# gabormarko/3D-semantic-segmentation

Measured on AMD Instinct MI355X. Metric: Mvoxel-views/sec, higher is better.
Workload: dtype f32; 1 GPU; R2: 200000 voxels x 300 views x 968x548x512 fp32 feature maps, room-shell scene seed 0, dmin 0.01 dmax 10 step 0.5*voxel; views_per_call=60, resident_feature_maps=60, parallelism=single GPU

## Files before the change

### 3d-semantic-segmentation_amd/csrc/voxproj.hip

```cpp
#include <hip/hip_runtime.h>

#include <cmath>
#include <cstdarg>
#include <cstdint>
#include <cstdio>
#include <cstdlib>
#include <cstring>
#include <algorithm>
#include <chrono>
#include <mutex>
#include <unordered_map>
#include <vector>

#include "voxproj.h"

#include "vp_common.h"
#include "vp_tables.h"
#include "vp_march.h"
#include "vp_gather.h"
#include "vp_aux.h"
#include "vp_prep.h"
#include "vp_aggregate.h"
#include "vp_render.h"
#include "vp_query.h"
#include "vp_splat.h"

#define VP_DISPATCH_KVU(KERNEL, VEC_OK, C, ...)                                   \
    do {                                                                          \
        if ((VEC_OK) == 2) hipLaunchKernelGGL((KERNEL<1, 8, VP_F16_U>), __VA_ARGS__);    \
        else if ((VEC_OK) && (C) > 256) hipLaunchKernelGGL((KERNEL<2, 4, 4>), __VA_ARGS__); \
        else if (VEC_OK) hipLaunchKernelGGL((KERNEL<1, 4, 4>), __VA_ARGS__);      \
        else hipLaunchKernelGGL((KERNEL<4, 1, 4>), __VA_ARGS__);                  \
    } while (0)
#define VP_DISPATCH_GATHER(G32, VEC_OK, C, ...)                                   \
    do {                                                                          \
        if ((VEC_OK) == 2) hipLaunchKernelGGL((k_gather<1, 8, VP_F16_U, GATHER_G16>), __VA_ARGS__);    \
        else if ((VEC_OK) && (C) > 256) hipLaunchKernelGGL((k_gather<2, 4, 4, G32>), __VA_ARGS__); \
        else if (VEC_OK) hipLaunchKernelGGL((k_gather<1, 4, 4, G32>), __VA_ARGS__);      \
        else hipLaunchKernelGGL((k_gather<4, 1, 4, 1>), __VA_ARGS__);               \
    } while (0)

#define VP_DISPATCH_GATHER_ONE(SMALL, VEC_OK, C, ...)                             \
    do {                                                                          \
        if ((VEC_OK) == 2) hipLaunchKernelGGL((k_gather_one<1, 8, VP_F16_U>), __VA_ARGS__);    \
        else if ((VEC_OK) && (C) > 256 && (SMALL)) hipLaunchKernelGGL((k_gather_one<2, 4, 8>), __VA_ARGS__); \
        else if ((VEC_OK) && (C) > 256) hipLaunchKernelGGL((k_gather_one<2, 4, 4>), __VA_ARGS__); \
        else if (VEC_OK) hipLaunchKernelGGL((k_gather_one<1, 4, 4>), __VA_ARGS__);      \
        else hipLaunchKernelGGL((k_gather_one<4, 1, 4>), __VA_ARGS__);                  \
    } while (0)

#ifndef VP_F16_U
#define VP_F16_U 4
#endif

extern "C" {

int vp_abi_version(void) { return VP_ABI_VERSION; }

const char *vp_last_error(void) { return g_err; }

size_t vp_workspace_bytes(int B, int V, int H, int W, int C, int dimz, int dimy, int dimx, int64_t n_rows)
{
    if (B <= 0 || V <= 0 || H <= 0 || W <= 0 || C <= 0 || n_rows <= 0 || dimz <= 0 || dimy <= 0 || dimx <= 0) return 0;
    return make_layout(B, V, H, W, C, n_rows, dimz, dimy, dimx).total;
}

static int workspace_status_impl(void *workspace, void *stream_, bool drain_all);

static int project_impl(const float *feats, bool feats_f16, const int64_t *occ, const float *vmi, const float *intr,
                        const float *opts_host, int32_t *count, float *out, int32_t *views_hit,
                        const float *grid_origin_host, float voxel_size,
                        int B, int V, int H, int W, int C, int dimz, int dimy, int dimx, int64_t n_rows,
                        void *workspace, size_t workspace_bytes, void *stream_, int flags, int32_t *ids_out = nullptr)
{
    const bool march_only = ids_out != nullptr;
    if (feats_f16 && (C % 8 != 0 || ((uintptr_t)feats & 15) != 0 || ((uintptr_t)out & 15) != 0))
        return fail(VP_EINVAL, "fp16 feature maps need C %% 8 == 0 and 16-byte aligned feats/out");
    if ((!march_only && (!feats || !count || !out)) || !occ || !vmi || !intr || !opts_host || !grid_origin_host || !workspace)
        return fail(VP_EINVAL, "null pointer argument");
    WsState *st = ws_state(workspace, true);
    struct HitGuard { WsState *st; bool keep; ~HitGuard() { if (!keep) st->has_hit = false; } } hit_guard{st, false};
    if (B <= 0 || V <= 0 || H <= 0 || W <= 0 || C <= 0 || dimz <= 0 || dimy <= 0 || dimx <= 0 || n_rows <= 0)
        return fail(VP_EINVAL, "non-positive dimension");
    if ((long long)B * V > 65535) return fail(VP_EINVAL, "B*V = %lld exceeds 65535", (long long)B * V);
    if ((long long)dimz * dimy * dimx >= (1ll << 31)) return fail(VP_EINVAL, "occupancy grid has >= 2^31 cells per batch");
    if ((long long)H * W >= (1ll << 31) || n_rows >= (1ll << 31)) return fail(VP_EINVAL, "image or row count >= 2^31");
    if ((flags & VP_FLAG_SYNC) && (flags & VP_FLAG_PIPELINE)) return fail(VP_EINVAL, "VP_FLAG_SYNC and VP_FLAG_PIPELINE exclude each other");
    Params p;
    p.width = (int)(opts_host[0] + 0.5f);
    p.height = (int)(opts_host[1] + 0.5f);
    if (p.width != W || p.height != H)
        return fail(VP_EINVAL, "opts width/height (%d,%d) must equal the feature map's (%d,%d)", p.width, p.height, W, H);
    p.dmin = opts_host[2]; p.dmax = opts_host[3]; p.inc = opts_host[4];
    if (!(p.inc > 0.0f)) return fail(VP_EINVAL, "rayIncrement must be > 0 (the reference would never terminate)");
    p.ox = grid_origin_host[0]; p.oy = grid_origin_host[1]; p.oz = grid_origin_host[2];
    p.vs = voxel_size;
    p.dimz = dimz; p.dimy = dimy; p.dimx = dimx;
    p.B = B; p.V = V; p.C = C; p.n_rows = n_rows;

    const Layout l = make_layout(B, V, H, W, C, n_rows, dimz, dimy, dimx, workspace_bytes);
    if (workspace_bytes < l.total) return fail(VP_EWORKSPACE, "workspace has %zu bytes, need %zu", workspace_bytes, l.total);
    if ((uintptr_t)workspace & 255) return fail(VP_EWORKSPACE, "workspace must be 256-byte aligned");
    if (!sticky_open(*st)) return fail(VP_EHIP, "could not allocate the workspace record's page of pinned host memory (sticky error words)");
    char *ws = (char *)workspace;
    hipStream_t s0 = (hipStream_t)stream_;

    const bool pipe = (flags & VP_FLAG_PIPELINE) != 0;
    PipeState *ps = &st->pipe;
    if (pipe && !pipe_open(*ps)) return fail(VP_EHIP, "could not create the side stream / events for VP_FLAG_PIPELINE");
    const bool gather_only = (flags & VP_FLAG_GATHER_ONLY) != 0;
    if (gather_only) {
        if (!st->has_hit || st->last_feats != (const void *)feats || st->last_f16 != feats_f16 || st->last_B != B || st->last_V != V ||
            st->last_H != H || st->last_W != W || st->last_C != C || st->B != B || st->dimz != dimz || st->dimy != dimy ||
            st->dimx != dimx || st->n_rows != n_rows || st->last_out != (const void *)out || st->last_count != (const void *)count ||
            st->last_vmi != (const void *)vmi)
            return fail(VP_EINVAL, "VP_FLAG_GATHER_ONLY repeats phase 2 of the previous call on this workspace: there is none (or it "
                                   "failed), or its feature maps / poses / outputs / shapes differ from this call's");
        if (st->opt_row_begin < 0 && st->opt_row_end < 0)
            return fail(VP_EINVAL, "VP_FLAG_GATHER_ONLY without a row range (VP_OPT_ROW_BEGIN / VP_OPT_ROW_END) would gather every row twice");
        if (!st->last_ranged)
            return fail(VP_EINVAL, "VP_FLAG_GATHER_ONLY after a call that had no row range: that call gathered every row already");
    }

    int q = 0;
    hipStream_t s1 = s0;
    if (gather_only) {
        q = st->last_q;
    } else if (pipe) {
        q = (int)(ps->calls & 1);
        s1 = ps->side;
    } else if (ps->ok && (ps->used[0] || ps->used[1])) {
        VP_HIP(hipStreamSynchronize(ps->side));
        ps->used[0] = ps->used[1] = false;
    }
    int *status = (int *)(ws + l.status[q]);
    int *cell_of_id = (int *)(ws + l.cell_of_id);
    unsigned long long *mask64 = (unsigned long long *)(ws + l.mask64);
    NearRec *near2 = (NearRec *)(ws + l.near2);
    unsigned char *dist = (unsigned char *)(ws + l.dist);
    unsigned char *dist_tmp = (unsigned char *)(ws + l.dist_tmp);
    int *cnt_call = (int *)(ws + l.cnt_call[q]);
    int *heavy_list = (int *)(ws + l.heavy[q]);
    int *work = (int *)(ws + l.work[q]);
    ViewEntry *viewtab = (ViewEntry *)(ws + l.viewtab[q]);
    int *hit = (int *)(ws + l.hit[q]);
    int *status0 = (int *)(ws + l.status[0]);

    const long long cells = (long long)dimz * dimy * dimx;
    int *occ_copy = (int *)(ws + l.occ_copy);
    WsState &rec = *st;
    const bool rec_matches = rec.B == B && rec.dimz == dimz && rec.dimy == dimy && rec.dimx == dimx && rec.n_rows == n_rows;
    const bool verify = (flags & VP_FLAG_VERIFY_ACCEL) && !pipe && !gather_only && !(flags & VP_FLAG_REUSE_ACCEL);
    const int cmp_blocks = (int)((cells * B + 255) / 256 > 8192 ? 8192 : (cells * B + 255) / 256);
    bool rebuild = !gather_only && !(flags & VP_FLAG_REUSE_ACCEL);
    if (!rebuild && !gather_only && (rec.builds == 0 || !rec_matches))
        return fail(VP_EINVAL, "VP_FLAG_REUSE_ACCEL, but this workspace holds no occupancy tables for a grid of this shape "
                               "(B, dims, n_rows): call once without the flag");
    if (rebuild || !rec.opened) {
        if (pipe && ps->ok) {
            VP_HIP(hipStreamSynchronize(ps->side));
        }
        hipLaunchKernelGGL(k_ws_open, dim3(1), dim3(64), 0, s0, status0, (int *)(ws + l.status[1]), WS_MAGIC, rec.gen, rebuild ? 1 : 0);
        rec.opened = true;
    }
    if (verify && rec_matches && rec.copy_valid) {
        volatile int *differs = rec.sticky_host + ST_OCCDIFF;
        *differs = 0;
        hipLaunchKernelGGL(k_occ_compare_copy, dim3(cmp_blocks), dim3(256), 0, s0, (const long long *)occ, occ_copy, cells * B, rec.sticky_dev + ST_OCCDIFF);
        VP_HIP(hipStreamSynchronize(s0));
        rebuild = *differs != 0;
    } else if (rebuild) {
        if (verify) {
            hipLaunchKernelGGL(k_occ_compare_copy, dim3(cmp_blocks), dim3(256), 0, s0, (const long long *)occ, occ_copy, cells * B, status + ST_OCCDIFF);
            rec.copy_valid = true;
        } else {
            rec.copy_valid = false;
        }
    }
    if (rebuild) {
        if (pipe) {
            VP_HIP(hipStreamSynchronize(ps->side));
            VP_HIP(hipStreamSynchronize(s0));
        }
        ProfSpan sp; sp.begin(0, s0);
        VP_HIP(hipMemsetAsync(cell_of_id, 0xFF, size_t(B) * n_rows * sizeof(int), s0));
        VP_HIP(hipMemsetAsync(mask64, 0, size_t(B) * l.nblk * sizeof(unsigned long long), s0));
        const int blocks = (int)((cells * B + 255) / 256 > 16384 ? 16384 : (cells * B + 255) / 256);
        hipLaunchKernelGGL(k_build_cells, dim3(blocks), dim3(256), 0, s0, (const long long *)occ, cell_of_id,
                           mask64, dimz, dimy, dimx, l.nby, l.nbx, l.nblk, B, (long long)n_rows);
        const int db = (int)(((long long)l.nbz * l.nby * l.nbx * B + 255) / 256);
        hipLaunchKernelGGL(k_block_dist, dim3(db), dim3(256), 0, s0, mask64, (const unsigned char *)nullptr, dist, l.nbz, l.nby, l.nbx, l.nblk, B, 0);
        hipLaunchKernelGGL(k_block_dist, dim3(db), dim3(256), 0, s0, mask64, (const unsigned char *)dist, dist_tmp, l.nbz, l.nby, l.nbx, l.nblk, B, 1);
        hipLaunchKernelGGL(k_block_dist, dim3(db), dim3(256), 0, s0, mask64, (const unsigned char *)dist_tmp, dist, l.nbz, l.nby, l.nbx, l.nblk, B, 2);
        const long long near_waves = (long long)l.nbz * l.nby * l.nbx * B;
        hipLaunchKernelGGL(k_build_near, dim3((unsigned)((near_waves + 3) / 4)), dim3(256), 0, s0, mask64, (const unsigned char *)dist,
                           near2, dimz, dimy, dimx, l.nbz, l.nby, l.nbx, l.nblk, B);
        rec.B = B; rec.dimz = dimz; rec.dimy = dimy; rec.dimx = dimx; rec.n_rows = n_rows;
        rec.builds++;
        hipLaunchKernelGGL(k_ws_seal, dim3(1), dim3(1), 0, s0, status0, tables_key(B, dimz, dimy, dimx, n_rows, rec.builds));
        sp.end();
        if (pipe) VP_HIP(hipStreamSynchronize(s0));
    }
    const unsigned expect_tables = tables_key(rec.B, rec.dimz, rec.dimy, rec.dimx, rec.n_rows, rec.builds);

    if (pipe && !gather_only) {
        if (ps->used[q]) VP_HIP(hipStreamWaitEvent(s1, ps->call_done[q], 0));
    }
    const bool ranged = rec.opt_row_begin >= 0 || rec.opt_row_end >= 0;
    const long long row_lo = std::max<long long>(1, rec.opt_row_begin);
    const long long row_hi = rec.opt_row_end < 0 ? (long long)n_rows : std::min<long long>(rec.opt_row_end, (long long)n_rows);

    int heavy_t = (int)std::min<long long>(256 + 64ll * B * V, 2048);
    if ((long long)B * V == 1) heavy_t = 256 + 64;
    if (rec.opt_heavy_t > 0) heavy_t = (int)std::min<long long>(rec.opt_heavy_t, 2147483647ll);
    if (flags & VP_FLAG_SERIAL_SUMS) heavy_t = 2147483647;
    const bool one_view = (long long)B * V == 1 && rec.opt_one_view != 0;
    PlanArgs plan;
    plan.heavy_t = heavy_t; plan.part_t = 2147483647; plan.part_px = 0; plan.count_heavy = 1; plan.dyn_px_min = 0; plan.dyn_t_ratio = 0;
    plan.dyn_t_floor = 0; plan.cell_in_item = 0;
    const long long px2 = 2ll * B * V * (long long)H * W;
    const bool one_split = one_view && heavy_t != 2147483647 && rec.opt_one_view_split != 0;
    if (!one_view && heavy_t != 2147483647) {
        long long ppx = rec.opt_part_px > 0 ? rec.opt_part_px : std::max<long long>(1, heavy_t);
        ppx = std::max(ppx, (px2 + l.slot_cap - 1) / l.slot_cap);
        plan.part_px = (int)std::min<long long>(ppx, 2147483647ll);
        heavy_t = std::max(heavy_t, plan.part_px);
        plan.heavy_t = plan.part_t = heavy_t;
    } else if (one_split) {
        const long long T = rec.opt_one_view_split > 0 ? rec.opt_one_view_split : rec.opt_heavy_t > 0 ? rec.opt_heavy_t : 0;
        long long ppx = rec.opt_part_px > 0 ? std::max(rec.opt_part_px, (px2 + l.slot_cap - 1) / l.slot_cap) : 0;
        if (ppx == 0 && T > 0) ppx = std::max<long long>((T + ONE_VIEW_T_RATIO - 1) / ONE_VIEW_T_RATIO, (px2 + l.slot_cap - 1) / l.slot_cap);
        plan.part_px = (int)std::min<long long>(ppx, 2147483646ll);
        plan.dyn_px_min = ppx > 0 ? 0 : ONE_VIEW_PART_MIN;
        plan.heavy_t = plan.part_t = T > 0 ? (int)std::min<long long>(std::max(T, ppx), 2147483646ll) : 0;
        plan.dyn_t_ratio = T > 0 ? 0 : ONE_VIEW_T_RATIO;
        plan.dyn_t_floor = (long long)H * W <= GATHER_G32_SMALL_IMAGE ? ONE_VIEW_T_FLOOR_SMALL : 0;
        plan.cell_in_item = 1;
        heavy_t = plan.heavy_t;
    } else if (one_view) {
        plan.count_heavy = 0;
    }
    static_assert(sizeof(PlanArgs) == sizeof(int) * 8, "PlanArgs is kept as ints in the workspace record");
    if (gather_only) { memcpy(&plan, st->last_plan, sizeof(plan)); heavy_t = plan.heavy_t; }
    const int part_px = plan.part_px;
    const bool plans_parts = part_px > 0 || plan.dyn_px_min > 0;
#ifdef VP_DIAG
    if (flags & VP_FLAG_DIAG_EVALS) heavy_t = -1;
    if (flags & VP_FLAG_DIAG_WAVES) heavy_t = -2;
#endif
    const int wl_blocks = (int)((n_rows + 256 * WL_PER_THREAD - 1) / (256 * WL_PER_THREAD));
    int4 *parts = (int4 *)(ws + l.parts[q]), *split = (int4 *)(ws + l.split[q]), *pmeta = (int4 *)(ws + l.pmeta[q]);
    float *prow = (float *)(ws + l.prow[q]);
    int *hit_waves = (int *)(ws + l.hitcnt[q]);
#define VP_LAUNCH_WORKLIST(STREAM)                                                                                              \
    hipLaunchKernelGGL(k_worklist, dim3((unsigned)(wl_blocks + (B * V + 255) / 256)), dim3(256), 0, STREAM, (const int *)cnt_call,   \
                       plan, (long long)n_rows, work, status, wl_blocks, vmi, viewtab, B * V, row_lo, row_hi, parts, split, \
                       (int)l.slot_cap, rec.sticky_dev, (const int *)cell_of_id, (const int *)hit_waves, (int)l.n_hitcnt)
    if (gather_only) {
        VP_HIP(hipMemsetAsync(status + ST_WORK0, 0, ST_PLAN_WORDS * sizeof(int), s0));
        VP_LAUNCH_WORKLIST(s0);
    }
    if (!gather_only) {
        ProfSpan sp; sp.begin(0, s1);
        hipLaunchKernelGGL(k_zero_call, dim3((unsigned)((n_rows + 1023) / 1024)), dim3(256), 0, s1, status, cnt_call, (long long)n_rows,
                           status0, rec.sticky_dev, WS_MAGIC, rec.gen, expect_tables, hit_waves,
                           (plan.dyn_px_min > 0 && !march_only) ? l.n_hitcnt : 0ll);
        sp.end();
    }
    if (!gather_only) {
        FirstHitArgs fa;
        fa.occ = (const long long *)occ; fa.vmi = vmi; fa.intr = intr; fa.near2 = near2; fa.dist = dist;
        fa.nby = l.nby; fa.nbx = l.nbx; fa.nblk = l.nblk; fa.hit = march_only ? (int *)ids_out : hit; fa.cnt_call = cnt_call;
        fa.heavy_list = heavy_list; fa.heavy_t = ((one_view && !one_split) || heavy_t < 0) ? heavy_t : 2147483647;
        fa.hit_waves = (plan.dyn_px_min > 0 && l.n_hitcnt > 0) ? hit_waves : nullptr;
        if (march_only) { fa.heavy_t = 2147483647; fa.hit_waves = nullptr; }
        fa.status = status; fa.sticky = rec.sticky_dev;
        const dim3 grid((W + 15) / 16, (H + 15) / 16, B * V);
        ProfSpan sp; sp.begin(1, s1);
        if (flags & VP_FLAG_EXACT_MARCH) {
            hipLaunchKernelGGL(k_first_hit<0>, grid, dim3(256), 0, s1, fa, p);
        } else {
            bool beside_gather = false;
            if (pipe && ps->used[q ^ 1]) {
                beside_gather = hipEventQuery(ps->call_done[q ^ 1]) == hipErrorNotReady;
                (void)hipGetLastError();
            }
            const size_t row_bytes = size_t(C) * (feats_f16 ? 2 : 4);
            size_t lds_req = beside_gather ? (row_bytes <= 1024 ? 30 : 41) * 1024 : 0;
            if (rec.opt_march_lds_kb >= 0) lds_req = size_t(std::min<long long>(rec.opt_march_lds_kb, 64)) * 1024;
            hipLaunchKernelGGL(k_first_hit<1>, grid, dim3(256), lds_req, s1, fa, p);
        }
        if (!march_only) VP_LAUNCH_WORKLIST(s1);
        sp.end();
    }
    if (march_only) {
        VP_HIP(hipGetLastError());
        ps->last_q = 0;
        if (flags & VP_FLAG_SYNC) return workspace_status_impl(workspace, stream_, true);
        return VP_OK;
    }
    if (pipe && !gather_only) VP_HIP(hipEventRecord(ps->fh_done[q], s1));

    GatherArgs g;
    g.feats = feats; g.hit = hit; g.viewtab = viewtab; g.intr = intr; g.cell_of_id = cell_of_id;
    g.cnt_call = cnt_call; g.heavy_list = heavy_list; g.n_heavy = status + ST_NHEAVY;
    g.row_lo = (int)row_lo; g.row_hi = (int)row_hi;
    g.work = work; g.work_n = status + ST_WORK0;
    g.parts = parts; g.split = split; g.pmeta = pmeta; g.prow = prow;
    g.host_word = nullptr; g.host_seq = 0;
    g.parts_on = (one_view && plans_parts) ? 1 : 0; g.slot_cap = (int)l.slot_cap; g.count = count; g.views_hit = views_hit; g.out = out; g.status = status;
    const int vec_ok = feats_f16 ? 2 : ((C % 4 == 0) && (((uintptr_t)feats & 15) == 0) && (((uintptr_t)out & 15) == 0)) ? 1 : 0;
    const bool small_image = (long long)B * V >= 8 && (long long)H * W <= GATHER_G32_SMALL_IMAGE;
    g.heavy_blocks = 0;
    if (pipe && !gather_only) VP_HIP(hipStreamWaitEvent(s0, ps->fh_done[q], 0));
    if (one_view) {
        ProfSpan sp; sp.begin(2, s0);
        const int per_cu = rec.opt_one_view > 0 ? (int)std::min<long long>(rec.opt_one_view, 256) : 16;
        const long long want = rec.opt_one_view >= 1000 ? rec.opt_one_view - 1000 : (long long)device_cus() * per_cu;
        const long long cap = (n_rows - 1 + 3) / 4;
        const unsigned nblk = (unsigned)std::max<long long>(1, std::min(want, cap));
        g.heavy_blocks = (heavy_t != 2147483647 && !plans_parts) ? (int)nblk : 0;
        volatile int *note = nullptr;
        if ((flags & VP_FLAG_SYNC) && plans_parts && n_rows > 1) {
            rec.split_seq = (rec.split_seq + 1) & 0x7fffu;
            note = rec.sticky_host + ST_HOST_NSPLIT;
            *note = 0;
            g.host_word = rec.sticky_dev + ST_HOST_NSPLIT; g.host_seq = (int)rec.split_seq;
        }
        if (n_rows > 1) VP_DISPATCH_GATHER_ONE((long long)H * W <= GATHER_G32_SMALL_IMAGE, vec_ok, C, dim3(nblk), dim3(256), 0, s0, g, p);
        sp.end();
        bool combine = n_rows > 1 && plans_parts;
        if (combine && note) {
            const auto t0 = std::chrono::steady_clock::now();
            for (unsigned spin = 0;; spin++) {
                const unsigned v = (unsigned)*note;
                if ((v >> 31) && ((v >> 16) & 0x7fffu) == rec.split_seq) { combine = (v & 0xffffu) != 0; break; }
                if ((spin & 63) == 63 && std::chrono::steady_clock::now() - t0 > std::chrono::milliseconds(2)) break;
                __builtin_ia32_pause();
            }
        }
        if (combine) {
            ProfSpan sc; sc.begin(3, s0);
            const dim3 cgrid((unsigned)std::max<long long>(1, std::min<long long>(COMBINE_BLOCKS, l.slot_cap / 2)));
            VP_DISPATCH_KVU(k_combine_parts, vec_ok, C, cgrid, dim3(256), 0, s0, g, p);
            sc.end();
        }
    } else if (n_rows > 1) {
        const long long items = (n_rows - 1) + (part_px > 0 ? std::min<long long>(l.slot_cap, px2 / part_px + 1) : 0);
        {
            ProfSpan sp; sp.begin(2, s0);
            const dim3 ggrid((unsigned)((items + 3) / 4));
            if (small_image) VP_DISPATCH_GATHER(4, vec_ok, C, ggrid, dim3(256), 0, s0, g, p);
            else VP_DISPATCH_GATHER(1, vec_ok, C, ggrid, dim3(256), 0, s0, g, p);
            sp.end();
        }
        if (part_px > 0) {
            ProfSpan sp; sp.begin(3, s0);
            const dim3 cgrid((unsigned)std::min<long long>(COMBINE_BLOCKS, std::max<long long>(1, l.slot_cap / 2)));
            VP_DISPATCH_KVU(k_combine_parts, vec_ok, C, cgrid, dim3(256), 0, s0, g, p);
            sp.end();
        }
    }
    if (pipe) {
        VP_HIP(hipEventRecord(ps->call_done[q], s0));
        ps->used[q] = true;
        ps->last_q = q;
        if (!gather_only) ps->calls++;
    } else if (!gather_only) {
        ps->last_q = 0;
    }
    VP_HIP(hipGetLastError());
    st->last_B = B; st->last_V = V; st->last_H = H; st->last_W = W; st->last_C = C; st->last_q = q;
    st->last_f16 = feats_f16; st->last_feats = (const void *)feats; st->last_out = (const void *)out; st->last_count = (const void *)count;
    st->last_vmi = (const void *)vmi; st->last_ranged = ranged; memcpy(st->last_plan, &plan, sizeof(plan));
    st->has_hit = true; st->hit_off = l.hit[q];
    hit_guard.keep = true;
    if (flags & VP_FLAG_SYNC) return workspace_status_impl(workspace, stream_, true);
    return VP_OK;
}

int vp_project_features(const float *feats, const int64_t *occ, const float *vmi, const float *intr,
                        const float *opts_host, int32_t *count, float *out, int32_t *views_hit,
                        const float *grid_origin_host, float voxel_size,
                        int B, int V, int H, int W, int C, int dimz, int dimy, int dimx, int64_t n_rows,
                        void *workspace, size_t workspace_bytes, void *stream_, int flags)
{
    return project_impl(feats, false, occ, vmi, intr, opts_host, count, out, views_hit, grid_origin_host, voxel_size,
                        B, V, H, W, C, dimz, dimy, dimx, n_rows, workspace, workspace_bytes, stream_, flags);
}

int vp_project_features_f16(const void *feats_f16, const int64_t *occ, const float *vmi, const float *intr,
                            const float *opts_host, int32_t *count, float *out, int32_t *views_hit,
                            const float *grid_origin_host, float voxel_size,
                            int B, int V, int H, int W, int C, int dimz, int dimy, int dimx, int64_t n_rows,
                            void *workspace, size_t workspace_bytes, void *stream_, int flags)
{
    return project_impl((const float *)feats_f16, true, occ, vmi, intr, opts_host, count, out, views_hit,
                        grid_origin_host, voxel_size, B, V, H, W, C, dimz, dimy, dimx, n_rows, workspace,
                        workspace_bytes, stream_, flags);
}

int vp_first_hit_ids(const int64_t *occ, const float *vmi, const float *intr, const float *opts_host,
                     const float *grid_origin_host, float voxel_size, int B, int V, int H, int W,
                     int dimz, int dimy, int dimx, int64_t n_rows, int32_t *ids,
                     void *workspace, size_t workspace_bytes, void *stream_, int flags)
{
    const int allowed = VP_FLAG_SYNC | VP_FLAG_REUSE_ACCEL | VP_FLAG_VERIFY_ACCEL | VP_FLAG_EXACT_MARCH;
    if (flags & ~allowed) return fail(VP_EINVAL, "vp_first_hit_ids accepts VP_FLAG_SYNC, _REUSE_ACCEL, _VERIFY_ACCEL and _EXACT_MARCH only (flags 0x%x)", flags);
    if (!ids) return fail(VP_EINVAL, "null pointer argument");
    return project_impl(nullptr, false, occ, vmi, intr, opts_host, nullptr, nullptr, nullptr, grid_origin_host, voxel_size,
                        B, V, H, W, 1, dimz, dimy, dimx, n_rows, workspace, workspace_bytes, stream_, flags, ids);
}

#ifndef RENDER_MAX_BLOCKS
#define RENDER_MAX_BLOCKS (1 << 20)
#endif

int vp_render_features(const int32_t *ids, int64_t n_pixels, const float *rows, int64_t n_rows, int C, void *dst,
                       int dst_is_f16, int32_t *bad_ids, void *stream_)
{
    if (!ids || !rows || !dst) return fail(VP_EINVAL, "null pointer argument");
    if (n_pixels <= 0 || n_rows <= 0 || C <= 0) return fail(VP_EINVAL, "non-positive dimension (n_pixels, n_rows or C)");
    hipStream_t stream = (hipStream_t)stream_;
    const long long tiles = (n_pixels + 63) / 64;
    const dim3 grid((unsigned)std::min<long long>((tiles + 3) / 4, RENDER_MAX_BLOCKS));
    const bool al16 = (((uintptr_t)rows | (uintptr_t)dst) & 15) == 0;
    int *bad = (int *)bad_ids;
#define VP_RENDER(KERNEL) hipLaunchKernelGGL(KERNEL, grid, dim3(256), 0, stream, (const int *)ids, (long long)n_pixels, rows, \
                                             (long long)n_rows, C, dst_t, bad)
    if (dst_is_f16) {
        _Float16 *dst_t = (_Float16 *)dst;
        if (C < 64) VP_RENDER((k_render_small<_Float16>));
        else if (C % 8 == 0 && al16) VP_RENDER((k_render_walk<8, 1, _Float16>));
        else VP_RENDER((k_render_walk<1, 4, _Float16>));
    } else {
        float *dst_t = (float *)dst;
        if (C < 64) VP_RENDER((k_render_small<float>));
        else if (C % 4 == 0 && al16) VP_RENDER((k_render_walk<4, 2, float>));
        else VP_RENDER((k_render_walk<1, 4, float>));
    }
#undef VP_RENDER
    VP_HIP(hipGetLastError());
    return VP_OK;
}

size_t vp_query_workspace_bytes(int P, int C)
{
    if (P < 1 || P > QUERY_MAX_P || C < 1 || C > QUERY_MAX_C) return 0;
    return align256((size_t)query_ppad(P) * query_cpad(C) * sizeof(float));
}

int vp_query_features(const void *rows, int rows_is_f16, int64_t n_rows, int C, int64_t row_stride, const float *text, int P,
                      float scale, float *logits, int32_t *labels, float *margin, int32_t *n_nonfinite, void *workspace,
                      size_t workspace_bytes, void *stream_)
{
    if (!rows || !labels || !text) return fail(VP_EINVAL, "null pointer argument (rows, labels or text)");
    if (n_rows < 1 || n_rows > INT32_MAX) return fail(VP_EINVAL, "n_rows = %lld outside [1, 2^31 - 1]", (long long)n_rows);
    if (C < 1 || C > QUERY_MAX_C) return fail(VP_EINVAL, "C = %d outside [1, %d]", C, QUERY_MAX_C);
    if (P < 1 || P > QUERY_MAX_P) return fail(VP_EINVAL, "P = %d outside [1, %d]", P, QUERY_MAX_P);
    if (row_stride < C) return fail(VP_EINVAL, "row_stride %lld < C = %d", (long long)row_stride, C);
    if (!(scale > 0.0f) || !std::isfinite(scale)) return fail(VP_EINVAL, "scale must be finite and > 0 (got %g)", (double)scale);
    const size_t need = vp_query_workspace_bytes(P, C);
    if (!workspace || workspace_bytes < need) return fail(VP_EWORKSPACE, "workspace has %zu bytes, need %zu", workspace ? workspace_bytes : 0, need);
    if ((uintptr_t)workspace & 255) return fail(VP_EWORKSPACE, "workspace must be 256-byte aligned");
    hipStream_t stream = (hipStream_t)stream_;
    const size_t esz = rows_is_f16 ? 2 : 4;
    const bool vec = C % (16 / esz) == 0 && ((uintptr_t)rows & 15) == 0 && ((size_t)row_stride * esz) % 16 == 0;
    const dim3 grid((unsigned)((n_rows + 16 * QUERY_WAVES - 1) / (16 * QUERY_WAVES))), block(64 * QUERY_WAVES);
#define VP_QUERY(T, VEC) hipLaunchKernelGGL((k_query<T, VEC, false>), grid, block, 0, stream, (const T *)rows, (long long)n_rows, C, \
                                            (long long)row_stride, (const T *)workspace, P, scale, logits, (int *)labels, margin, \
                                            (int *)n_nonfinite)
#define VP_QUERY1(T) hipLaunchKernelGGL((k_query<T, true, true>), grid, block, 0, stream, (const T *)rows, (long long)n_rows, C, \
                                        (long long)row_stride, (const T *)workspace, P, scale, logits, (int *)labels, margin, \
                                        (int *)n_nonfinite)
    if (rows_is_f16) {
        hipLaunchKernelGGL((k_query_text<_Float16>), dim3(query_ppad(P)), dim3(64), 0, stream, text, P, C, (_Float16 *)workspace);
        if (vec && C <= QUERY_NS * QueryTraits<_Float16>::W) VP_QUERY1(_Float16);
        else if (vec) VP_QUERY(_Float16, true);
        else VP_QUERY(_Float16, false);
    } else {
        hipLaunchKernelGGL((k_query_text<float>), dim3(query_ppad(P)), dim3(64), 0, stream, text, P, C, (float *)workspace);
        if (vec && C <= QUERY_NS * QueryTraits<float>::W) VP_QUERY1(float);
        else if (vec) VP_QUERY(float, true);
        else VP_QUERY(float, false);
    }
#undef VP_QUERY
#undef VP_QUERY1
    VP_HIP(hipGetLastError());
    return VP_OK;
}

size_t vp_splat_workspace_bytes(int64_t n_gaussians, int W, int H, int64_t capacity)
{
    if (n_gaussians < 0 || n_gaussians > INT32_MAX || W < 1 || W > SPLAT_MAX_WH || H < 1 || H > SPLAT_MAX_WH || capacity < 0 ||
        capacity > INT32_MAX)
        return 0;
    SplatLayout l;
    return splat_layout(n_gaussians, W, H, capacity, l) ? l.bytes : 0;
}

int vp_splat_project(const float *means, const float *quats, const float *scales, const float *opacities, int64_t n_gaussians,
                     const float *viewmat, float fx, float fy, float cx, float cy, int W, int H, float near_plane,
                     float far_plane, float eps2d, int64_t *n_isect, int32_t *n_nonfinite, void *workspace,
                     size_t workspace_bytes, void *stream_)
{
    if (n_gaussians < 0 || n_gaussians > INT32_MAX)
        return fail(VP_EINVAL, "n_gaussians = %lld outside [0, 2^31 - 1]", (long long)n_gaussians);
    if (n_gaussians > 0 && (!means || !quats || !scales || !opacities))
        return fail(VP_EINVAL, "null pointer argument (means, quats, scales or opacities)");
    if (!viewmat) return fail(VP_EINVAL, "null viewmat");
    if (W < 1 || W > SPLAT_MAX_WH || H < 1 || H > SPLAT_MAX_WH)
        return fail(VP_EINVAL, "image %d x %d outside [1, %d]^2", W, H, SPLAT_MAX_WH);
    for (int k = 0; k < 12; ++k)
        if (!std::isfinite(viewmat[k])) return fail(VP_EINVAL, "viewmat[%d] is not finite", k);
    if (!(fx > 0.0f) || !(fy > 0.0f) || !std::isfinite(fx) || !std::isfinite(fy) || !std::isfinite(cx) || !std::isfinite(cy))
        return fail(VP_EINVAL, "fx, fy must be finite and > 0, cx, cy finite (got %g %g %g %g)", (double)fx, (double)fy,
                    (double)cx, (double)cy);
    if (!(near_plane > 0.0f) || !(far_plane > near_plane) || !(eps2d >= 0.0f) || !std::isfinite(eps2d))
        return fail(VP_EINVAL, "need 0 < near < far and a finite eps2d >= 0 (got %g %g %g)", (double)near_plane,
                    (double)far_plane, (double)eps2d);
    if (!workspace) return fail(VP_EWORKSPACE, "workspace is NULL");
    if ((uintptr_t)workspace & 255) return fail(VP_EWORKSPACE, "workspace must be 256-byte aligned");
    SplatLayout l;
    if (!splat_layout(n_gaussians, W, H, 0, l)) return fail(VP_EHIP, "rocprim scratch size query failed");
    if (workspace_bytes < l.bytes) return fail(VP_EWORKSPACE, "workspace has %zu bytes, need %zu", workspace_bytes, l.bytes);
    hipStream_t stream = (hipStream_t)stream_;
    char *ws = (char *)workspace;
    SplatCam cam;
    for (int k = 0; k < 12; ++k) cam.r[k] = viewmat[k];
    cam.fx = fx; cam.fy = fy; cam.cx = cx; cam.cy = cy;
    cam.near_z = near_plane; cam.far_z = far_plane; cam.eps2d = eps2d;
    cam.W = W; cam.H = H; cam.tiles_x = l.tiles_x;
    long long *total = (long long *)(ws + l.total), *offs = (long long *)(ws + l.offs);
    if (n_gaussians > 0) {
        hipLaunchKernelGGL(k_splat_project, dim3((unsigned)((n_gaussians + 255) / 256)), dim3(256), 0, stream, means, quats,
                           scales, opacities, (long long)n_gaussians, cam, (SplatRec *)(ws + l.rec), (int4 *)(ws + l.box),
                           (int *)(ws + l.count), (int *)n_nonfinite);
        VP_HIP(hipGetLastError());
        size_t tmp = l.scan_bytes;
        VP_HIP(rocprim::inclusive_scan(ws + l.scan_tmp, tmp, (const int *)(ws + l.count), offs, (size_t)n_gaussians,
                                       rocprim::plus<long long>(), stream));
    }
    hipLaunchKernelGGL(k_splat_total, dim3(1), dim3(1), 0, stream, (const long long *)offs, (long long)n_gaussians, total,
                       (long long *)n_isect);
    VP_HIP(hipGetLastError());
    return VP_OK;
}

int vp_splat_rasterize(const float *features, int D, int64_t row_stride, int64_t n_gaussians, int W, int H, int64_t capacity,
                       int32_t *labels, float *confidence, float *alpha, float *logits, int32_t *status, void *workspace,
                       size_t workspace_bytes, void *stream_)
{
    if (n_gaussians < 0 || n_gaussians > INT32_MAX)
        return fail(VP_EINVAL, "n_gaussians = %lld outside [0, 2^31 - 1]", (long long)n_gaussians);
    if (!labels || (n_gaussians > 0 && !features)) return fail(VP_EINVAL, "null pointer argument (labels or features)");
    if (D < 1 || D > SPLAT_MAX_D) return fail(VP_EINVAL, "D = %d outside [1, %d]", D, SPLAT_MAX_D);
    if (row_stride < D) return fail(VP_EINVAL, "row_stride %lld < D = %d", (long long)row_stride, D);
    if (W < 1 || W > SPLAT_MAX_WH || H < 1 || H > SPLAT_MAX_WH)
        return fail(VP_EINVAL, "image %d x %d outside [1, %d]^2", W, H, SPLAT_MAX_WH);
    if (capacity < 0 || capacity > INT32_MAX) return fail(VP_EINVAL, "capacity = %lld outside [0, 2^31 - 1]", (long long)capacity);
    if (!workspace) return fail(VP_EWORKSPACE, "workspace is NULL");
    if ((uintptr_t)workspace & 255) return fail(VP_EWORKSPACE, "workspace must be 256-byte aligned");
    SplatLayout l;
    if (!splat_layout(n_gaussians, W, H, capacity, l)) return fail(VP_EHIP, "rocprim scratch size query failed");
    if (workspace_bytes < l.bytes) return fail(VP_EWORKSPACE, "workspace has %zu bytes, need %zu", workspace_bytes, l.bytes);
    hipStream_t stream = (hipStream_t)stream_;
    char *ws = (char *)workspace;
    const long long n_tiles = (long long)l.tiles_x * l.tiles_y;
    const long long *total = (const long long *)(ws + l.total);
    unsigned long long *k0 = (unsigned long long *)(ws + l.keys0), *k1 = (unsigned long long *)(ws + l.keys1);
    int *v0 = (int *)(ws + l.vals0), *v1 = (int *)(ws + l.vals1);
    longlong2 *ranges = (longlong2 *)(ws + l.ranges);
    const long long n_emit = std::max<long long>(n_gaussians, 1);
    const unsigned g_emit = (unsigned)((n_emit + 255) / 256);
    hipLaunchKernelGGL(k_splat_emit, dim3(g_emit), dim3(256), 0, stream, (const SplatRec *)(ws + l.rec),
                       (const int4 *)(ws + l.box), (const long long *)(ws + l.offs), (long long)n_gaussians, l.tiles_x,
                       n_tiles, total, (long long)capacity, k0, v0, (int *)status);
    VP_HIP(hipGetLastError());
    if (capacity > 0) {
        size_t tmp = l.sort_bytes;
        VP_HIP(rocprim::radix_sort_pairs(ws + l.sort_tmp, tmp, k0, k1, v0, v1, (size_t)capacity, 0u, (unsigned)l.end_bit,
                                         stream));
    }
    VP_HIP(hipMemsetAsync(ranges, 0, (size_t)n_tiles * sizeof(longlong2), stream));
    if (capacity > 0) {
        hipLaunchKernelGGL(k_splat_ranges, dim3((unsigned)((capacity + 255) / 256)), dim3(256), 0, stream, k1, total,
                           (long long)capacity, ranges);
        VP_HIP(hipGetLastError());
    }
    const dim3 grid((unsigned)l.tiles_x, (unsigned)l.tiles_y), block(SPLAT_THREADS);
#define VP_SPLAT(DT) hipLaunchKernelGGL((k_splat_blend<DT>), grid, block, 0, stream, (const SplatRec *)(ws + l.rec), v1, ranges, \
                                        total, (long long)capacity, features, D, (long long)row_stride, W, H, (int *)labels, \
                                        confidence, alpha, logits)
    if (D <= 8) VP_SPLAT(8);
    else if (D <= 16) VP_SPLAT(16);
    else if (D <= 32) VP_SPLAT(32);
    else VP_SPLAT(64);
#undef VP_SPLAT
    VP_HIP(hipGetLastError());
    return VP_OK;
}

static int read_status(void *workspace, hipStream_t stream, int *st )
{
// ... 324 lines not shown
```

### 3d-semantic-segmentation_amd/csrc/vp_march.h

```cpp
#pragma once

namespace {

struct FirstHitArgs {
    const long long *occ;
    const float *vmi;
    const float *intr;
    const NearRec *near2;
    const unsigned char *dist;
    int nby, nbx;
    long long nblk;
    int *hit;
    int *cnt_call;
    int *heavy_list;
    int heavy_t;
    int *hit_waves;
    int *status;
    int *sticky;
};

struct MarchView {
    const long long *occ_b;
    const NearRec *near_b;
    const unsigned char *dist_b;
    int nby, nbx;
    float cpx, cpy, cpz;
    float fx, fy, mx, my, fw, fh;
    float rvs;
};

struct MarchRay {
    float cdx, cdy, cdz;
    float wdx, wdy, wdz;
    float tEnd;
    float inv_dcell;
    float thr;
    bool leap_ok;
};

struct MarchBlock {
    unsigned cur_blk = 0xffffffffu;
    int cur_d = 0;
    unsigned long long p0 = 0ull, p1 = 0ull, p2 = 0ull;
};

struct MarchBinade {
    float bT2 = 0.0f, bTu = 0.0f, bg = 0.0f, brg = 0.0f;
};

__device__ __forceinline__ int march_sample(const Params &p, const MarchView &mv, const MarchRay &r, MarchBlock &mb, float t, int &D)
{
    const float px = mv.cpx + t * r.wdx, py = mv.cpy + t * r.wdy, pz = mv.cpz + t * r.wdz;
    const float ax = px - p.ox, ay = py - p.oy, az = pz - p.oz;
    const float qx = ax * mv.rvs, qy = ay * mv.rvs, qz = az * mv.rvs;
    const float rx = rintf(qx), ry = rintf(qy), rz = rintf(qz);
    const bool safe = (fabsf(qx - rx) < r.thr) & (fabsf(qy - ry) < r.thr) & (fabsf(qz - rz) < r.thr);
    int ix = (int)rx, iy = (int)ry, iz = (int)rz;
    if (__builtin_expect(!safe, 0)) {
        ix = f2i_sat(round_half_away(ax / p.vs));
        iy = f2i_sat(round_half_away(ay / p.vs));
        iz = f2i_sat(round_half_away(az / p.vs));
    }
    D = 0;
    const bool ing = ((unsigned)ix < (unsigned)p.dimx) & ((unsigned)iy < (unsigned)p.dimy) & ((unsigned)iz < (unsigned)p.dimz);
    if (__builtin_expect(ing, 1)) {
        const unsigned blk = ((unsigned)(iz >> 2) * (unsigned)mv.nby + (unsigned)(iy >> 2)) * (unsigned)mv.nbx + (unsigned)(ix >> 2);
        if (blk != mb.cur_blk) {
            mb.cur_blk = blk;
            const NearRec n3 = mv.near_b[blk];
            mb.cur_d = (int)n3.dist;
            mb.p0 = n3.p0; mb.p1 = n3.p1; mb.p2 = n3.p2;
        }
        const int bit = ((iz & 3) << 4) | ((iy & 3) << 2) | (ix & 3);
        const int nd = (int)((mb.p0 >> bit) & 1ull) | ((int)((mb.p1 >> bit) & 1ull) << 1) | ((int)((mb.p2 >> bit) & 1ull) << 2);
        D = mb.cur_d <= 1 ? nd : (mb.cur_d - 1) * 4 + 1;
        if (__builtin_expect((mb.cur_d <= 1) & (nd == 0), 0)) {
            const float camx = r.cdx * t, camy = r.cdy * t, camz = r.cdz * t;
            const float u = mv.fx * (camx / camz) + mv.mx;
            const float v = mv.fy * (camy / camz) + mv.my;
            if ((u >= 0.0f) && (u < mv.fw) && (v >= 0.0f) && (v < mv.fh))
                return (int)mv.occ_b[((long long)iz * p.dimy + iy) * p.dimx + ix];
        }
    } else if (r.leap_ok) {
        const int lim = 1 << 29;
        const int jx = min(max(ix, -lim), lim), jy = min(max(iy, -lim), lim), jz = min(max(iz, -lim), lim);
        const int ex = jx < 0 ? -jx : (jx >= p.dimx ? jx - p.dimx + 1 : 0);
        const int ey = jy < 0 ? -jy : (jy >= p.dimy ? jy - p.dimy + 1 : 0);
        const int ez = jz < 0 ? -jz : (jz >= p.dimz ? jz - p.dimz + 1 : 0);
        const int dbox = max(ex, max(ey, ez));
        const int kx = min(max(jx, 0), p.dimx - 1), ky = min(max(jy, 0), p.dimy - 1), kz = min(max(jz, 0), p.dimz - 1);
        const int cb_ = ((kz >> 2) * mv.nby + (ky >> 2)) * mv.nbx + (kx >> 2);
        const int dd = mv.dist_b[cb_];
        const int din = dd > 0 ? (dd - 1) * 4 + 1 : 0;
        D = max(dbox, din - dbox);
    }
    return 0;
}

__device__ __forceinline__ int march_steps(const MarchRay &r, int D)
{
    return 1 + (D >= 2 ? (int)fminf(((float)D - 1.5f) * r.inv_dcell, 16777216.0f) : 0);
}

__device__ __forceinline__ void march_advance(float inc, float tEnd, MarchBinade &bn, float &t, int S)
{
    for (;;) {
        if (t >= bn.bT2) {
            const unsigned eb = __float_as_uint(t) & 0x7f800000u;
            const float T = __uint_as_float(eb);
            const float u = __uint_as_float(eb - (23u << 23));
            bn.bT2 = __uint_as_float(eb + (1u << 23));
            bn.bTu = bn.bT2 - u;
            bn.bg = (T + inc) - T;
            const float r = inc - bn.bg;
            const bool fast = (t > 0.0f) & (eb >= (30u << 23)) & (eb < (0xfeu << 23)) & (inc < T) & (bn.bg > 0.0f) & (fabsf(r) * 2.0f != u);
            bn.brg = fast ? __builtin_amdgcn_rcpf(bn.bg) * 0.999999f : 0.0f;
        }
        const int m = (int)fminf(fmaxf((bn.bTu - t) * bn.brg, 0.0f), (float)S);
        t = t + (float)m * bn.bg;
        S -= m;
        if (S <= 0) break;
        t += inc;
        S -= 1;
        if (S <= 0 || !(t < tEnd)) break;
    }
}

template <int MODE>
__device__ __forceinline__ void first_hit_body(const FirstHitArgs &fa, const Params &p, int x, int y, int bv)
{
    constexpr bool ACCEL = MODE != 0;
    const long long *__restrict__ occ = fa.occ;
    const float *__restrict__ vmi = fa.vmi;
    const float *__restrict__ intr = fa.intr;
    const long long nblk = fa.nblk;
    int *__restrict__ hit = fa.hit;
    int *cnt_call = fa.cnt_call, *heavy_list = fa.heavy_list, *status = fa.status;
    const int heavy_t = fa.heavy_t;
    const int b = bv / p.V;
#ifdef VP_DIAG
    const unsigned long long dbg_t0 = __builtin_amdgcn_s_memrealtime();
    int dbg_it = 0;
#endif
    if (x >= p.width || y >= p.height) return;
    if (status[ST_STALE]) return;

    const float *m = vmi + (long long)bv * 16;
    const float fx = intr[b * 4 + 0], fy = intr[b * 4 + 1], mx = intr[b * 4 + 2], my = intr[b * 4 + 3];

    const float depth = 1.0f * (p.dmax - p.dmin) + p.dmin;
    const float sx = ((float)(unsigned)x - mx) / fx;
    const float sy = ((float)(unsigned)y - my) / fy;
    float cx = depth * sx, cy = depth * sy, cz = depth;
    float inv = 1.0f / sqrtf(cx * cx + cy * cy + cz * cz);
    const float cdx = cx * inv, cdy = cy * inv, cdz = cz * inv;
    const float cpx = m[0] * 0.0f + m[1] * 0.0f + m[2] * 0.0f + m[3] * 1.0f;
    const float cpy = m[4] * 0.0f + m[5] * 0.0f + m[6] * 0.0f + m[7] * 1.0f;
    const float cpz = m[8] * 0.0f + m[9] * 0.0f + m[10] * 0.0f + m[11] * 1.0f;
    float wx = m[0] * cdx + m[1] * cdy + m[2] * cdz + m[3] * 0.0f;
    float wy = m[4] * cdx + m[5] * cdy + m[6] * cdz + m[7] * 0.0f;
    float wz = m[8] * cdx + m[9] * cdy + m[10] * cdz + m[11] * 0.0f;
    inv = 1.0f / sqrtf(wx * wx + wy * wy + wz * wz);
    const float wdx = wx * inv, wdy = wy * inv, wdz = wz * inv;

    const float d2r = 1.0f / cdz;
    float t = d2r * p.dmin;
    const float tEnd = d2r * p.dmax;
    const long long cells = (long long)p.dimz * p.dimy * p.dimx;
    const long long *occ_b = occ + (long long)b * cells;
    const float fw = (float)p.width, fh = (float)p.height;
    int id = 0;
    if ((t < tEnd) && !(tEnd + p.inc > tEnd)) {
        atomicOr(&status[ST_STUCK], 1);
        *(volatile int *)&fa.sticky[ST_STICKY_STUCK] = 1;
        t = tEnd;
    }
    if constexpr (!ACCEL) {
        while (t < tEnd) {
            const float px = cpx + t * wdx, py = cpy + t * wdy, pz = cpz + t * wdz;
            const int ix = f2i_sat(round_half_away((px - p.ox) / p.vs));
            const int iy = f2i_sat(round_half_away((py - p.oy) / p.vs));
            const int iz = f2i_sat(round_half_away((pz - p.oz) / p.vs));
            const float camx = cdx * t, camy = cdy * t, camz = cdz * t;
            const float u = fx * (camx / camz) + mx;
            const float v = fy * (camy / camz) + my;
            const bool inb = (u >= 0.0f) && (u < fw) && (v >= 0.0f) && (v < fh);
            if (inb && ix >= 0 && iy >= 0 && iz >= 0 && ix < p.dimx && iy < p.dimy && iz < p.dimz) {
                id = (int)occ_b[((long long)iz * p.dimy + iy) * p.dimx + ix];
                if (id != 0) break;
            }
            t += p.inc;
        }
    } else {
        MarchView mv;
        mv.occ_b = occ_b;
        mv.near_b = fa.near2 + (long long)b * nblk;
        mv.dist_b = fa.dist + (long long)b * nblk;
        mv.nby = fa.nby; mv.nbx = fa.nbx;
        mv.cpx = cpx; mv.cpy = cpy; mv.cpz = cpz;
        mv.fx = fx; mv.fy = fy; mv.mx = mx; mv.my = my; mv.fw = fw; mv.fh = fh;
        mv.rvs = 1.0f / p.vs;
        MarchRay r;
        r.cdx = cdx; r.cdy = cdy; r.cdz = cdz; r.wdx = wdx; r.wdy = wdy; r.wdz = wdz; r.tEnd = tEnd;
        const float dcell = fabsf(p.inc * mv.rvs) * fmaxf(fabsf(wdx), fmaxf(fabsf(wdy), fabsf(wdz))) * 1.01f + 1e-6f;
        const float span = (fabsf(cpx) + fabsf(cpy) + fabsf(cpz) + fabsf(p.ox) + fabsf(p.oy) + fabsf(p.oz) + fabsf(tEnd)) * fabsf(mv.rvs);
        r.leap_ok = (span < 131072.0f) & (fabsf(tEnd) < 1.0e5f * fabsf(p.inc)) & (dcell == dcell) & (dcell < 1.0e6f);
        r.inv_dcell = r.leap_ok ? 0.999f / dcell : 0.0f;
        r.thr = r.leap_ok ? 0.5f - span * 0x1p-21f : -1.0f;
        MarchBlock mb;
        MarchBinade bn;
#ifdef VP_DIAG
        int dbg_leap = 0, dbg_fine = 0;
#endif
        while (t < tEnd) {
            int D;
            id = march_sample(p, mv, r, mb, t, D);
            if (id != 0) break;
#ifdef VP_DIAG
            if (heavy_t < 0) { if (D >= 2) dbg_leap++; else dbg_fine++; }
            dbg_it++;
#endif
            march_advance(p.inc, tEnd, bn, t, march_steps(r, D));
        }
#ifdef VP_DIAG
        if (heavy_t == -2) {
            const unsigned long long t1 = __builtin_amdgcn_s_memrealtime();
            const int l = threadIdx.x & 63;
            const int mine = dbg_leap + dbg_fine;
            for (int off = 32; off > 0; off >>= 1) dbg_it = max(dbg_it, __shfl_xor(dbg_it, off));
            hit[((long long)bv * p.height + y) * p.width + x] = l == 0 ? (int)(unsigned)dbg_t0 : l == 1 ? (int)(unsigned)t1 : l == 2 ? dbg_it : mine;
            return;
        }
        if (heavy_t < 0) {
            hit[((long long)bv * p.height + y) * p.width + x] = (min(dbg_leap, 1023) << 10) | min(dbg_fine, 1023);
            return;
        }
#endif
    }
    if (id != 0 && (id < 0 || id >= p.n_rows)) {
        atomicOr(&status[ST_BADID], 1);
        *(volatile int *)&fa.sticky[ST_STICKY_BADID] = 1;
        id = 0;
    }
    hit[((long long)bv * p.height + y) * p.width + x] = id;
    {
        const int lane_ = threadIdx.x & 63;
        int my_n = 0;
        unsigned long long todo = __ballot(id != 0);
        if (fa.hit_waves && todo != 0ull && lane_ == __builtin_ctzll(todo))
            fa.hit_waves[((long long)blockIdx.y * gridDim.x + blockIdx.x) * 4 + (threadIdx.x >> 6)] = __popcll(todo);
        while (todo) {
            const int l = __builtin_ctzll(todo);
            const int cur = __builtin_amdgcn_readlane(id, l);
            const unsigned long long m = __ballot(id == cur);
            if (lane_ == l) my_n = __popcll(m);
            todo &= ~m;
        }
        if (my_n > 0) {
            const int old = atomicAdd(&cnt_call[id], my_n);
            if (old <= heavy_t && old + my_n > heavy_t) heavy_list[atomicAdd(&status[ST_NHEAVY], 1)] = id;
        }
    }
}

template <int MODE>
__global__ __launch_bounds__(256) void k_first_hit(FirstHitArgs fa, Params p)
{
    const int wave = threadIdx.x >> 6, lane = threadIdx.x & 63;
    const int x = blockIdx.x * 16 + (wave & 1) * 8 + (lane & 7);
    const int y = blockIdx.y * 16 + (wave >> 1) * 8 + (lane >> 3);
    first_hit_body<MODE>(fa, p, x, y, blockIdx.z);
}

}
```

Baseline: 1116 Mvoxel-views/s.

## Remap first-hit march blocks across XCDs and specialize heavy-list enlistment

Result: no change. 1132 Mvoxel-views/s (median of 6 runs) (+1.5%).

```diff
diff --git a/3d-semantic-segmentation_amd/csrc/voxproj.hip b/3d-semantic-segmentation_amd/csrc/voxproj.hip
--- a/3d-semantic-segmentation_amd/csrc/voxproj.hip
+++ b/3d-semantic-segmentation_amd/csrc/voxproj.hip
@@ -51,6 +51,43 @@
 
 #ifndef VP_F16_U
 #define VP_F16_U 4
+#endif
+
+#ifdef VP_SHADOW_MARCH
+struct ShadowScratch { char *p = nullptr; size_t bytes = 0; };
+static ShadowScratch g_shadow;
+
+static int shadow_march_launch(dim3 grid, size_t lds_req, hipStream_t s, const int64_t *occ, const float *vmi, const float *intr,
+                               const NearRec *near2, const unsigned char *dist, const Layout &l, long long pixels, long long n_rows,
+                               int *sticky, const Params &p)
+{
+    if (VP_SHADOW_MARCH == 0) return VP_OK;
+    const size_t need = align256(size_t(pixels) * 4) + align256(size_t(n_rows) * 4) + 256 * 4;
+    if (g_shadow.bytes < need) {
+        VP_HIP(hipDeviceSynchronize());
+        if (g_shadow.p) VP_HIP(hipFree(g_shadow.p));
+        g_shadow.p = nullptr; g_shadow.bytes = 0;
+        VP_HIP(hipMalloc((void **)&g_shadow.p, need));
+        VP_HIP(hipMemset(g_shadow.p, 0, need));
+        g_shadow.bytes = need;
+    }
+    int *hit = (int *)g_shadow.p;
+    int *cnt = (int *)(g_shadow.p + align256(size_t(pixels) * 4));
+    int *status = (int *)(g_shadow.p + align256(size_t(pixels) * 4) + align256(size_t(n_rows) * 4));
+    FirstHitArgs fa;
+    fa.occ = (const long long *)occ; fa.vmi = vmi; fa.intr = intr; fa.near2 = near2; fa.dist = dist;
+    fa.nby = l.nby; fa.nbx = l.nbx; fa.nblk = l.nblk; fa.hit = hit; fa.cnt_call = cnt; fa.heavy_list = status + 128;
+    fa.heavy_t = 2147483647; fa.hit_waves = nullptr; fa.status = status; fa.sticky = sticky;
+    switch (VP_SHADOW_MARCH) {
+    case 1: hipLaunchKernelGGL((k_first_hit<1, false, 0>), grid, dim3(256), lds_req, s, fa, p); break;
+    case 2: hipLaunchKernelGGL((k_first_hit<1, false, 1>), grid, dim3(256), lds_req, s, fa, p); break;
+    case 3: hipLaunchKernelGGL((k_first_hit<1, false, 2>), grid, dim3(256), lds_req, s, fa, p); break;
+    case 4: hipLaunchKernelGGL((k_first_hit<1, false, 3>), grid, dim3(256), lds_req, s, fa, p); break;
+    default: hipLaunchKernelGGL(k_march_spin, grid, dim3(256), lds_req, s, status, 1.0f); break;
+    }
+    VP_HIP(hipGetLastError());
+    return VP_OK;
+}
 #endif
 
 extern "C" {
@@ -277,8 +314,10 @@
         fa.status = status; fa.sticky = rec.sticky_dev;
         const dim3 grid((W + 15) / 16, (H + 15) / 16, B * V);
         ProfSpan sp; sp.begin(1, s1);
+        const bool enlist = fa.heavy_t != 2147483647;
         if (flags & VP_FLAG_EXACT_MARCH) {
-            hipLaunchKernelGGL(k_first_hit<0>, grid, dim3(256), 0, s1, fa, p);
+            if (enlist) hipLaunchKernelGGL((k_first_hit<0, true>), grid, dim3(256), 0, s1, fa, p);
+            else hipLaunchKernelGGL((k_first_hit<0, false>), grid, dim3(256), 0, s1, fa, p);
         } else {
             bool beside_gather = false;
             if (pipe && ps->used[q ^ 1]) {
@@ -288,7 +327,14 @@
             const size_t row_bytes = size_t(C) * (feats_f16 ? 2 : 4);
             size_t lds_req = beside_gather ? (row_bytes <= 1024 ? 30 : 41) * 1024 : 0;
             if (rec.opt_march_lds_kb >= 0) lds_req = size_t(std::min<long long>(rec.opt_march_lds_kb, 64)) * 1024;
-            hipLaunchKernelGGL(k_first_hit<1>, grid, dim3(256), lds_req, s1, fa, p);
+#ifdef VP_SHADOW_MARCH
+            if (pipe) {
+                if (ps->used[q ^ 1]) VP_HIP(hipStreamWaitEvent(s1, ps->call_done[q ^ 1], 0));
+                lds_req = 0;
+            }
+#endif
+            if (enlist) hipLaunchKernelGGL((k_first_hit<1, true>), grid, dim3(256), lds_req, s1, fa, p);
+            else hipLaunchKernelGGL((k_first_hit<1, false>), grid, dim3(256), lds_req, s1, fa, p);
         }
         if (!march_only) VP_LAUNCH_WORKLIST(s1);
         sp.end();
@@ -300,6 +346,14 @@
         return VP_OK;
     }
     if (pipe && !gather_only) VP_HIP(hipEventRecord(ps->fh_done[q], s1));
+#ifdef VP_SHADOW_MARCH
+    if (pipe && !gather_only && !(flags & VP_FLAG_EXACT_MARCH)) {
+        const dim3 grid((W + 15) / 16, (H + 15) / 16, B * V);
+        const size_t lds_req = size_t(C) * (feats_f16 ? 2 : 4) <= 1024 ? 30 * 1024 : 41 * 1024;
+        int rc = shadow_march_launch(grid, lds_req, s1, occ, vmi, intr, near2, dist, l, (long long)B * V * H * W, n_rows, rec.sticky_dev, p);
+        if (rc != VP_OK) return rc;
+    }
+#endif
 
     GatherArgs g;
     g.feats = feats; g.hit = hit; g.viewtab = viewtab; g.intr = intr; g.cell_of_id = cell_of_id;
diff --git a/3d-semantic-segmentation_amd/csrc/vp_march.h b/3d-semantic-segmentation_amd/csrc/vp_march.h
--- a/3d-semantic-segmentation_amd/csrc/vp_march.h
+++ b/3d-semantic-segmentation_amd/csrc/vp_march.h
@@ -127,24 +127,22 @@
 }
 
 template <int MODE>
-__device__ __forceinline__ void first_hit_body(const FirstHitArgs &fa, const Params &p, int x, int y, int bv)
+__device__ __forceinline__ int first_hit_march(const FirstHitArgs &fa, const Params &p, int x, int y, int bv, bool &done)
 {
     constexpr bool ACCEL = MODE != 0;
     const long long *__restrict__ occ = fa.occ;
     const float *__restrict__ vmi = fa.vmi;
     const float *__restrict__ intr = fa.intr;
     const long long nblk = fa.nblk;
-    int *__restrict__ hit = fa.hit;
-    int *cnt_call = fa.cnt_call, *heavy_list = fa.heavy_list, *status = fa.status;
-    const int heavy_t = fa.heavy_t;
+    int *__restrict__ status = fa.status;
     const int b = bv / p.V;
 #ifdef VP_DIAG
+    int *__restrict__ hit = fa.hit;
+    const int heavy_t = fa.heavy_t;
     const unsigned long long dbg_t0 = __builtin_amdgcn_s_memrealtime();
     int dbg_it = 0;
 #endif
-    if (x >= p.width || y >= p.height) return;
-    if (status[ST_STALE]) return;
-
+    done = false;
     const float *m = vmi + (long long)bv * 16;
     const float fx = intr[b * 4 + 0], fy = intr[b * 4 + 1], mx = intr[b * 4 + 2], my = intr[b * 4 + 3];
 
@@ -229,11 +227,13 @@
             const int mine = dbg_leap + dbg_fine;
             for (int off = 32; off > 0; off >>= 1) dbg_it = max(dbg_it, __shfl_xor(dbg_it, off));
             hit[((long long)bv * p.height + y) * p.width + x] = l == 0 ? (int)(unsigned)dbg_t0 : l == 1 ? (int)(unsigned)t1 : l == 2 ? dbg_it : mine;
-            return;
+            done = true;
+            return 0;
         }
         if (heavy_t < 0) {
             hit[((long long)bv * p.height + y) * p.width + x] = (min(dbg_leap, 1023) << 10) | min(dbg_fine, 1023);
-            return;
+            done = true;
+            return 0;
         }
 #endif
     }
@@ -242,34 +242,87 @@
         *(volatile int *)&fa.sticky[ST_STICKY_BADID] = 1;
         id = 0;
     }
-    hit[((long long)bv * p.height + y) * p.width + x] = id;
-    {
-        const int lane_ = threadIdx.x & 63;
-        int my_n = 0;
-        unsigned long long todo = __ballot(id != 0);
-        if (fa.hit_waves && todo != 0ull && lane_ == __builtin_ctzll(todo))
-            fa.hit_waves[((long long)blockIdx.y * gridDim.x + blockIdx.x) * 4 + (threadIdx.x >> 6)] = __popcll(todo);
-        while (todo) {
-            const int l = __builtin_ctzll(todo);
-            const int cur = __builtin_amdgcn_readlane(id, l);
-            const unsigned long long m = __ballot(id == cur);
-            if (lane_ == l) my_n = __popcll(m);
-            todo &= ~m;
-        }
+    return id;
+}
+
+template <bool ENLIST>
+__device__ __forceinline__ void first_hit_histogram(const FirstHitArgs &fa, int id, int tile_xy)
+{
+    const int lane_ = threadIdx.x & 63;
+    int my_n = 0;
+    unsigned long long todo = __ballot(id != 0);
+    if (fa.hit_waves && todo != 0ull && lane_ == __builtin_ctzll(todo))
+        fa.hit_waves[(long long)tile_xy * 4 + (threadIdx.x >> 6)] = __popcll(todo);
+    while (todo) {
+        const int l = __builtin_ctzll(todo);
+        const int cur = __builtin_amdgcn_readlane(id, l);
+        const unsigned long long m = __ballot(id == cur);
+        if (lane_ == l) my_n = __popcll(m);
+        todo &= ~m;
+    }
+    if constexpr (ENLIST) {
         if (my_n > 0) {
-            const int old = atomicAdd(&cnt_call[id], my_n);
-            if (old <= heavy_t && old + my_n > heavy_t) heavy_list[atomicAdd(&status[ST_NHEAVY], 1)] = id;
-        }
-    }
-}
-
-template <int MODE>
+            const int old = atomicAdd(&fa.cnt_call[id], my_n);
+            if (old <= fa.heavy_t && old + my_n > fa.heavy_t) fa.heavy_list[atomicAdd(&fa.status[ST_NHEAVY], 1)] = id;
+        }
+    } else {
+        if (my_n > 0) (void)atomicAdd(&fa.cnt_call[id], my_n);
+    }
+}
+
+template <int MODE, bool ENLIST, int ARM = 0>
+__device__ __forceinline__ void first_hit_body(const FirstHitArgs &fa, const Params &p, int x, int y, int bv, int tile_xy)
+{
+    const bool live = x < p.width && y < p.height && !fa.status[ST_STALE];
+    int id = 0;
+    if (live) {
+        bool done;
+        id = first_hit_march<MODE>(fa, p, x, y, bv, done);
+        if (done) return;
+        if constexpr (!(ARM & 2)) fa.hit[((long long)bv * p.height + y) * p.width + x] = id;
+    }
+    if constexpr (!(ARM & 1)) first_hit_histogram<ENLIST>(fa, id, tile_xy);
+}
+
+struct MarchTile { int tx, ty, bv; };
+__device__ __forceinline__ MarchTile march_tile()
+{
+#ifdef VP_MARCH_NO_XCD_REMAP
+    return {(int)blockIdx.x, (int)blockIdx.y, (int)blockIdx.z};
+#else
+    const unsigned gx = gridDim.x, gy = gridDim.y, n = gx * gy * gridDim.z;
+    const unsigned L = blockIdx.x + gx * (blockIdx.y + gy * blockIdx.z);
+    const unsigned x8 = L % 8u, q = n / 8u, r = n % 8u;
+    const unsigned T = x8 * q + min(x8, r) + L / 8u;
+    const unsigned row = T / gx;
+    return {(int)(T - row * gx), (int)(row % gy), (int)(row / gy)};
+#endif
+}
+
+template <int MODE, bool ENLIST, int ARM = 0>
 __global__ __launch_bounds__(256) void k_first_hit(FirstHitArgs fa, Params p)
 {
     const int wave = threadIdx.x >> 6, lane = threadIdx.x & 63;
-    const int x = blockIdx.x * 16 + (wave & 1) * 8 + (lane & 7);
-    const int y = blockIdx.y * 16 + (wave >> 1) * 8 + (lane >> 3);
-    first_hit_body<MODE>(fa, p, x, y, blockIdx.z);
-}
-
-}
+    const MarchTile t = march_tile();
+    const int x = t.tx * 16 + (wave & 1) * 8 + (lane & 7);
+    const int y = t.ty * 16 + (wave >> 1) * 8 + (lane >> 3);
+    first_hit_body<MODE, ENLIST, ARM>(fa, p, x, y, t.bv, t.ty * (int)gridDim.x + t.tx);
+}
+
+
+#ifdef VP_SHADOW_MARCH
+#ifndef VP_SPIN_ITERS
+#define VP_SPIN_ITERS 400
+#endif
+__global__ __launch_bounds__(256) void k_march_spin(int *sink, float seed)
+{
+    float a = seed + (float)threadIdx.x, b = a + 1.0f, c = a + 2.0f, d = a + 3.0f;
+    for (int i = 0; i < VP_SPIN_ITERS; i++) {
+        a = fmaf(a, 0.999f, 0.5f); b = fmaf(b, 0.999f, 0.25f); c = fmaf(c, 0.999f, 0.125f); d = fmaf(d, 0.999f, 0.0625f);
+    }
+    const float r = a + b + c + d;
+    if (r != r) sink[threadIdx.x] = 1;
+}
+#endif
+
+}
```
